# TUMFTM/CamRaDepth

Hardware: AMD Instinct MI355X
Metric: training images/sec at 256x416 bf16 (higher is better)
Workload: dtype bf16; 1 GPU; CamRaDepth base (image+radar) train step, 8x7x256x416 per GPU, bf16 MFMA / fp32 accumulate, diffGradNorm + OneCycleLR, Dropout2d/DropPath on; global_batch=8, parallelism=dp1, hip_graph=True

## Files before the change

camradepth_amd/csrc/encoder_ops.hip:

```cpp
#include <stdlib.h>
#include "common.h"

namespace {

constexpr int TPB = 256;

constexpr int DTH = 8;
constexpr int DCW = 64;

struct InNorm {
  const crd_sum_t* stats;
  const float* gamma; const float* beta; int gmul;
};
__device__ __forceinline__ void innorm_coeffs(const InNorm& n, int b, int C, long long P, int c0, bool ok, float (&a)[8], float (&s)[8]) {
#pragma unroll
  for (int j = 0; j < 8; ++j) { a[j] = 1.f; s[j] = 0.f; }
  if (n.stats == nullptr || !ok) return;
  float mean, rstd;
  const int grp = (c0 >> 4) / n.gmul;
  gn_mean_rstd(n.stats + (long long)b * (C >> 4) * 2, grp * n.gmul, n.gmul, (float)P * 16.f * n.gmul, mean, rstd);
#pragma unroll
  for (int j = 0; j < 8; ++j) {
    a[j] = n.gamma[c0 + j] * rstd;
    s[j] = n.beta[c0 + j] - mean * a[j];
// ... 97 lines not shown
  float s = 0.f, ss = 0.f;
  float rs0[8], rs1[8], rmean = 0.f, rrstd = 0.f;
#pragma unroll
  for (int j = 0; j < 8; ++j) rs0[j] = rs1[j] = 0.f;
  if (red.xr && gok) gn_mean_rstd(red.stats + (long long)b * (C >> 4) * 2, c0 >> 4, 1, (float)H * W * 16.f, rmean, rrstd);
#pragma unroll
  for (int i = 0; i < ROWS; ++i) {
#pragma unroll
    for (int kx = 0; kx < 3; ++kx) lds8(r0 + i + 2, xc + kx, win[(i + 2) % 3][kx]);
    const int oy = ty0 + r0 + i, ox = tx0 + xc;
    f32x2 acc[4];
#pragma unroll
    for (int q = 0; q < 4; ++q) acc[q] = bv[q];
#pragma unroll
    for (int ky = 0; ky < 3; ++ky)
#pragma unroll
      for (int kx = 0; kx < 3; ++kx) {
#pragma unroll
        for (int q = 0; q < 4; ++q) acc[q] = __builtin_elementwise_fma(win[(i + ky) % 3][kx][q], wv[ky * 3 + kx][q], acc[q]);
      }
    if (gok && oy < H && ox < W) {
      uint4 u;
      u.x = pack_bf2(acc[0][0], acc[0][1]); u.y = pack_bf2(acc[1][0], acc[1][1]); u.z = pack_bf2(acc[2][0], acc[2][1]); u.w = pack_bf2(acc[3][0], acc[3][1]);
      *reinterpret_cast<uint4*>(yb + ((long long)oy * W + ox) * C + c0) = u;
      if (red.xr) {
        const uint4 xv = xrv[i];
        const float gq[8] = {bf_lo(u.x), bf_hi(u.x), bf_lo(u.y), bf_hi(u.y), bf_lo(u.z), bf_hi(u.z), bf_lo(u.w), bf_hi(u.w)};
        const float xq[8] = {bf_lo(xv.x), bf_hi(xv.x), bf_lo(xv.y), bf_hi(xv.y), bf_lo(xv.z), bf_hi(xv.z), bf_lo(xv.w), bf_hi(xv.w)};
#pragma unroll
        for (int j = 0; j < 8; ++j) { rs0[j] += gq[j]; rs1[j] += gq[j] * ((xq[j] - rmean) * rrstd); }
      }
      if (STATS) {
        s += bf_lo(u.x) + bf_hi(u.x) + bf_lo(u.y) + bf_hi(u.y) + bf_lo(u.z) + bf_hi(u.z) + bf_lo(u.w) + bf_hi(u.w);
        ss += bf_lo(u.x) * bf_lo(u.x) + bf_hi(u.x) * bf_hi(u.x) + bf_lo(u.y) * bf_lo(u.y) + bf_hi(u.y) * bf_hi(u.y) +
              bf_lo(u.z) * bf_lo(u.z) + bf_hi(u.z) * bf_hi(u.z) + bf_lo(u.w) * bf_lo(u.w) + bf_hi(u.w) * bf_hi(u.w);
      }
    }
  }
  if (STATS) {
    s += __shfl_xor(s, 1); ss += __shfl_xor(ss, 1);
#pragma unroll
    for (int o = 8; o < 64; o <<= 1) { s += __shfl_xor(s, o); ss += __shfl_xor(ss, o); }
    const int wave = t >> 6, l = t & 63;
    if (l < 8 && (l & 1) == 0) { sred[wave][(l >> 1) * 2] = s; sred[wave][(l >> 1) * 2 + 1] = ss; }
    __syncthreads();
    if (t < 8) {
      const float v = sred[0][t] + sred[1][t] + sred[2][t] + sred[3][t];
      const int slab = (c_win >> 4) + (t >> 1);
      if (slab < (C >> 4)) stat_add(&stats[((long long)b * (C >> 4) + slab) * 2 + (t & 1)], v);
    }
  }
  if (red.xr) {
#pragma unroll
    for (int o = 8; o < 64; o <<= 1) {
#pragma unroll
      for (int j = 0; j < 8; ++j) { rs0[j] += __shfl_xor(rs0[j], o); rs1[j] += __shfl_xor(rs1[j], o); }
    }
    __syncthreads();
    float* fr = reinterpret_cast<float*>(sh);
    const int wave = t >> 6, l = t & 63;
    if (l < 8) {
#pragma unroll
      for (int j = 0; j < 8; ++j) { fr[wave * 128 + (l * 8 + j) * 2] = rs0[j]; fr[wave * 128 + (l * 8 + j) * 2 + 1] = rs1[j]; }
    }
    __syncthreads();
    const int nch = nG * 8;
    if (t < 2 * nch) {
      const float v = fr[t] + fr[128 + t] + fr[256 + t] + fr[384 + t];
      const int c = c_win + (t >> 1);
      grad_add(&red.r[((long long)b * C + c) * 2 + (t & 1)], v);
      fr[512 + t] = v * red.gamma[c];
    }
    __syncthreads();
    if (t < 2 * (nch >> 4)) {
      const int grp = t >> 1, which = t & 1;
      float a = 0.f;
#pragma unroll
      for (int j = 0; j < 16; ++j) a += fr[512 + (grp * 16 + j) * 2 + which];
      grad_add(&red.r[(long long)gridDim.z * C * 2 + ((long long)b * (C >> 4) + (c_win >> 4) + grp) * 2 + which], a);
    }
  }
}

#ifndef CRD_DWW_WGS
#define CRD_DWW_WGS 2
#endif
template <int TW>
__global__ __launch_bounds__(TPB, CRD_DWW_WGS) void k_dwconv_wgrad(const bf16_t* x, const bf16_t* dy, int H, int W, int C, crd_sum_t* dw10,
                                                      int replicas, int tiles_x, int tiles_y, int tiles_per_wg, InNorm inn) {
  constexpr int HWD = TW + 2;
  constexpr int HPX = (DTH + 2) * HWD;
  constexpr int RSPLIT = 32 / TW;
  constexpr int ROWS = DTH / RSPLIT;
  extern __shared__ __attribute__((aligned(16))) uint4 dsm[];
  uint4* sx = dsm;
  uint4* sdy = dsm + HPX * 8;
  const int b = blockIdx.z;
  const int c_win = blockIdx.y * DCW;
  const int txi = blockIdx.x % tiles_x, ygrp = blockIdx.x / tiles_x;
  const int tx0 = txi * TW;
  const bf16_t* xb = x + (long long)b * H * W * C;
  const bf16_t* db = dy + (long long)b * H * W * C;
  const int t = threadIdx.x;
  const int nG = (C - c_win) >= DCW ? 8 : (C - c_win) >> 3;
  const int g = t & 7, xc = (t >> 3) % TW, rg = (t >> 3) / TW;
  float acc[10][8];
#pragma unroll
  for (int tp = 0; tp < 10; ++tp)
#pragma unroll
    for (int j = 0; j < 8; ++j) acc[tp][j] = 0.f;
  float na[8], ns[8];
  for (int it = 0; it < tiles_per_wg; ++it) {
    const int tyi = ygrp * tiles_per_wg + it;
    if (tyi >= tiles_y) break;
    const int ty0 = tyi * DTH;
    {
      constexpr int NX = (HPX * 8 + TPB - 1) / TPB, ND = (DTH * TW * 8) / TPB;
      uint4 rx[NX], rd[ND];
      bool inimg[NX];
#pragma unroll
      for (int k = 0; k < NX; ++k) {
        const int i = t + k * TPB;
        const int hp = i >> 3, gg = i & 7;
        const int hy = hp / HWD, hx = hp - hy * HWD;
        const int iy = ty0 - 1 + hy, ix = tx0 - 1 + hx;
        inimg[k] = i < HPX * 8 && gg < nG && (unsigned)iy < (unsigned)H && (unsigned)ix < (unsigned)W;
        const int cy = iy < 0 ? 0 : (iy < H ? iy : H - 1), cx = ix < 0 ? 0 : (ix < W ? ix : W - 1), cgr = gg < nG ? gg : 0;
        const uint4 u = *reinterpret_cast<const uint4*>(xb + ((long long)cy * W + cx) * C + c_win + cgr * 8);
        rx[k] = inimg[k] ? u : make_uint4(0, 0, 0, 0);
      }
#pragma unroll
      for (int k = 0; k < ND; ++k) {
        const int i = t + k * TPB;
        const int pp = i >> 3, gg = i & 7;
        const int py = pp / TW, px = pp - py * TW;
        const int iy = ty0 + py, ix = tx0 + px;
        const int cy = iy < H ? iy : H - 1, cx = ix < W ? ix : W - 1, cgr = gg < nG ? gg : 0;
        const uint4 u = *reinterpret_cast<const uint4*>(db + ((long long)cy * W + cx) * C + c_win + cgr * 8);
        rd[k] = (gg < nG && iy < H && ix < W) ? u : make_uint4(0, 0, 0, 0);
      }
      if (it == 0) innorm_coeffs(inn, b, C, (long long)H * W, c_win + (t & 7) * 8, (t & 7) < nG, na, ns);
      if (it > 0) __syncthreads();
#pragma unroll
      for (int k = 0; k < NX; ++k) {
        const int i = t + k * TPB;
        if (i < HPX * 8) sx[i] = (inn.stats && inimg[k]) ? innorm_apply(rx[k], na, ns) : rx[k];
      }
#pragma unroll
      for (int k = 0; k < ND; ++k) sdy[t + k * TPB] = rd[k];
    }
    __syncthreads();
    float win[3][3][8];
    const int r0 = rg * ROWS;
#pragma unroll
    for (int ky = 0; ky < 2; ++ky)
#pragma unroll
      for (int kx = 0; kx < 3; ++kx) unpack8(sx[((r0 + ky) * HWD + xc + kx) * 8 + g], win[ky][kx]);
#pragma unroll
    for (int i = 0; i < ROWS; ++i) {
#pragma unroll
      for (int kx = 0; kx < 3; ++kx) unpack8(sx[((r0 + i + 2) * HWD + xc + kx) * 8 + g], win[(i + 2) % 3][kx]);
      float d[8];
      unpack8(sdy[((r0 + i) * TW + xc) * 8 + g], d);
#pragma unroll
      for (int j = 0; j < 8; ++j) acc[9][j] += d[j];
#pragma unroll
      for (int ky = 0; ky < 3; ++ky)
#pragma unroll
        for (int kx = 0; kx < 3; ++kx) {
#pragma unroll
          for (int j = 0; j < 8; ++j) acc[ky * 3 + kx][j] += d[j] * win[(i + ky) % 3][kx][j];
        }
    }
  }
#pragma unroll
  for (int o = 8; o < 64; o <<= 1) {
#pragma unroll
    for (int tp = 0; tp < 10; ++tp)
#pragma unroll
      for (int j = 0; j < 8; ++j) acc[tp][j] += __shfl_xor(acc[tp][j], o);
  }
  __syncthreads();
  float* sm = reinterpret_cast<float*>(dsm);
  const int wave = t >> 6, l = t & 63;
  for (int w = 0; w < 4; ++w) {
    if (wave == w && l < 8) {
#pragma unroll
      for (int tp = 0; tp < 10; ++tp)
#pragma unroll
        for (int j = 0; j < 8; ++j) {
          float* p = &sm[tp * 64 + l * 8 + j];
          *p = w == 0 ? acc[tp][j] : *p + acc[tp][j];
        }
    }
    __syncthreads();
  }
  crd_sum_t* dst = dw10 + (long long)((blockIdx.z * gridDim.x + blockIdx.x) % replicas) * 10 * C;
  const int nch = nG * 8;
  for (int i = t; i < 10 * nch; i += TPB) {
    const int tp = i / nch, cl = i - tp * nch;
    const float v = sm[tp * 64 + cl];
    if (v != 0.f) grad_add(&dst[(long long)tp * C + c_win + cl], v);
  }
}

}

static int dw_tile_width(int W) {
  static int forced = -1;
  if (forced < 0) forced = crd_dev_int("CRD_DW_TW", 0);
  if (forced == 16 || forced == 32) return forced;
  return W <= 16 ? 16 : 32;
}

extern "C" int crd_dwconv3x3(const void* x, int32_t B, int32_t H, int32_t W, int32_t C, const float* w9, const float* bias,
                             int32_t flip, void* y, crd_sum_t* stats, const crd_sum_t* in_stats, int32_t in_gmul,
                             const float* in_gamma, const float* in_beta, const void* red_x, const crd_sum_t* red_stats,
                             const float* red_gamma, crd_sum_t* red_r, crd_stream_t stream) {
  CRD_CHECK_ARG(x && w9 && y, "crd_dwconv3x3: null pointer");
  CRD_CHECK_ARG(!red_x || (red_stats && red_gamma && red_r), "crd_dwconv3x3: incomplete fused-reduce arguments");
  const RedOut red{reinterpret_cast<const bf16_t*>(red_x), red_stats, red_gamma, red_r};
  CRD_CHECK_ARG(!in_stats || (in_gamma && in_beta && in_gmul >= 1 && (C / 16) % in_gmul == 0), "crd_dwconv3x3: bad input-norm arguments");
  const InNorm inn{in_stats, in_gamma, in_beta, in_gmul};
  CRD_CHECK_ARG(C % 16 == 0, "crd_dwconv3x3: C must be a multiple of 16");
  const bf16_t* xp = reinterpret_cast<const bf16_t*>(x);
  bf16_t* yp = reinterpret_cast<bf16_t*>(y);
  hipStream_t st = as_stream(stream);
  const int tw = dw_tile_width(W);
  const int tiles_x = cdiv(W, tw), tiles_y = cdiv(H, DTH);
  dim3 grid(tiles_x * tiles_y, cdiv(C, DCW), B);
#define CRD_DW(FL, STT, TWV) hipLaunchKernelGGL((k_dwconv<FL, STT, TWV>), grid, dim3(TPB), 0, st, xp, H, W, C, w9, bias, yp, stats, tiles_x, inn, red)
  if (tw == 32) {
    if (flip) { if (stats) CRD_DW(true, true, 32); else CRD_DW(true, false, 32); }
    else { if (stats) CRD_DW(false, true, 32); else CRD_DW(false, false, 32); }
  } else {
    if (flip) { if (stats) CRD_DW(true, true, 16); else CRD_DW(true, false, 16); }
    else { if (stats) CRD_DW(false, true, 16); else CRD_DW(false, false, 16); }
  }
#undef CRD_DW
  CRD_LAUNCH_CHECK("crd_dwconv3x3");
  return CRD_OK;
}

extern "C" int crd_dwconv3x3_wgrad(const void* x, const void* dy, int32_t B, int32_t H, int32_t W, int32_t C, crd_sum_t* dw10,
                                   int32_t replicas, const crd_sum_t* in_stats, int32_t in_gmul, const float* in_gamma,
                                   const float* in_beta, crd_stream_t stream) {
  CRD_CHECK_ARG(x && dy && dw10 && replicas >= 1, "crd_dwconv3x3_wgrad: null pointer / replicas < 1");
  CRD_CHECK_ARG(!in_stats || (in_gamma && in_beta && in_gmul >= 1 && (C / 16) % in_gmul == 0), "crd_dwconv3x3_wgrad: bad input-norm arguments");
  const InNorm inn{in_stats, in_gamma, in_beta, in_gmul};
  CRD_CHECK_ARG(C % 16 == 0 && C <= 4096, "crd_dwconv3x3_wgrad: C must be a multiple of 16, <= 4096");
  const int tw = dw_tile_width(W);
  const int tiles_x = cdiv(W, tw), tiles_y = cdiv(H, DTH), wins = cdiv(C, DCW);
  int ysplit = cdiv(512, (long long)tiles_x * wins * B);
  if (ysplit > tiles_y) ysplit = tiles_y;
  if (ysplit < 1) ysplit = 1;
  const int per = cdiv(tiles_y, ysplit);
  ysplit = cdiv(tiles_y, per);
  dim3 grid(tiles_x * ysplit, wins, B);
  const bf16_t* xp = reinterpret_cast<const bf16_t*>(x);
  const bf16_t* dp = reinterpret_cast<const bf16_t*>(dy);
  hipStream_t st = as_stream(stream);
  if (tw == 32) {
    const size_t lds = (size_t)((DTH + 2) * 34 * 8 + DTH * 32 * 8) * sizeof(uint4);
    crd_reserve_lds_once<&k_dwconv_wgrad<32>>((int)lds, "k_dwconv_wgrad");
    hipLaunchKernelGGL(k_dwconv_wgrad<32>, grid, dim3(TPB), lds, st, xp, dp, H, W, C, dw10, replicas, tiles_x, tiles_y, per, inn);
  } else {
    const size_t lds = (size_t)((DTH + 2) * 18 * 8 + DTH * 16 * 8) * sizeof(uint4);
    crd_reserve_lds_once<&k_dwconv_wgrad<16>>((int)lds, "k_dwconv_wgrad");
    hipLaunchKernelGGL(k_dwconv_wgrad<16>, grid, dim3(TPB), lds, st, xp, dp, H, W, C, dw10, replicas, tiles_x, tiles_y, per, inn);
  }
  CRD_LAUNCH_CHECK("crd_dwconv3x3_wgrad");
  return CRD_OK;
}
```

camradepth_amd/lib.py:

```python
import ctypes as C
import os
import struct

import torch

_HERE = os.path.dirname(os.path.abspath(__file__))
LIB_PATH = os.environ.get("CRD_LIB") or os.path.join(_HERE, "libcamradepth_hip.so")


class CrdError(RuntimeError):
    pass


class ConvDesc(C.Structure):
    _fields_ = [
        ("x", C.c_void_p), ("x_ld", C.c_int32), ("x_coff", C.c_int32),
        ("B", C.c_int32), ("IH", C.c_int32), ("IW", C.c_int32), ("Cin", C.c_int32),
        ("w", C.c_void_p), ("Cout", C.c_int32), ("KH", C.c_int32), ("KW", C.c_int32),
        ("stride", C.c_int32), ("pad", C.c_int32), ("OH", C.c_int32), ("OW", C.c_int32),
        ("gather_mode", C.c_int32),
        ("y", C.c_void_p), ("y_ld", C.c_int32), ("y_coff", C.c_int32), ("y_f32", C.c_int32),
        ("out_mode", C.c_int32), ("patch_k", C.c_int32), ("patch_c", C.c_int32),
        ("bias", C.c_void_p), ("bias_bstride", C.c_int32), ("act", C.c_int32),
        ("res", C.c_void_p), ("res_ld", C.c_int32), ("res_scale", C.c_void_p),
# ... 26 lines not shown
        ("dw", C.c_void_p), ("dbias", C.c_void_p), ("dw_partials", C.c_void_p), ("dw_partial_capacity", C.c_int32), ("wg_budget", C.c_int32),
    ]


class WgradGroupInfo(C.Structure):
    _fields_ = [("n_problems", C.c_int32), ("n_items", C.c_int32 * 4), ("item_offset", C.c_int32 * 4), ("bytes", C.c_int64)]


class PackEntry(C.Structure):
    _fields_ = [
        ("src", C.c_void_p), ("dst_fwd", C.c_void_p), ("dst_dgrad", C.c_void_p), ("dst_scatter", C.c_void_p),
        ("cmap", C.c_void_p),
        ("Cout", C.c_int32), ("Cin_ref", C.c_int32), ("taps", C.c_int32), ("Cin_pad", C.c_int32),
        ("Cout_pad", C.c_int32), ("dst_f32", C.c_int32),
        ("dgrad_ld", C.c_int32), ("dgrad_coff", C.c_int32), ("dgrad_row0", C.c_int32), ("dgrad_rows", C.c_int32),
    ]


class MlpDesc(C.Structure):
    _fields_ = [(n, C.c_void_p) for n in ("x1", "x1_stats", "norm_gamma", "norm_beta", "w_fc1", "b_fc1", "norm1_gamma", "norm1_beta",
                                          "w9", "b_dw", "norm2_gamma", "norm2_beta", "w_fc2", "xn", "h1", "h2", "h3", "h1_stats",
                                          "h2_stats", "fc2_partials")] + \
               [(n, C.c_int32) for n in ("B", "H", "W", "C", "hidden")]


class UnpackEntry(C.Structure):
    _fields_ = [
        ("src", C.c_void_p), ("dst", C.c_void_p), ("cmap", C.c_void_p),
        ("Cout", C.c_int32), ("Cin_ref", C.c_int32), ("taps", C.c_int32), ("Cin_pad", C.c_int32),
        ("replicas", C.c_int32), ("src_sum", C.c_int32), ("replica_stride", C.c_int64),
    ]


class DgnDesc(C.Structure):
    _fields_ = [(n, C.c_void_p) for n in ("p", "g", "exp_avg", "exp_avg_sq", "prev_grad", "exp_grad_norm", "factor", "parts", "seg_off",
                                          "blk2seg", "blk2chunk", "active", "hp_dev", "gate", "clip", "ema")] + \
               [("parts_stride", C.c_int64), ("n_tensors", C.c_int32), ("n_blocks", C.c_int32)] + \
               [(n, C.c_float) for n in ("lr", "beta1", "beta2", "eps", "weight_decay")] + \
               [("step", C.c_int32), ("max_norm", C.c_float), ("ema_decay", C.c_float),
                ("ema_warmup", C.c_int32), ("ema_n", C.c_int32), ("ema_base", C.c_int32)]


_lib = None
ABI_VERSION = 13


def load():
    global _lib
    if _lib is not None:
        return _lib
    if not os.path.exists(LIB_PATH):
        raise CrdError(f"{LIB_PATH} is missing: run `python -m camradepth_amd.build` (hipcc, gfx950). "
                       "camradepth_amd has no CPU fallback.")
    lib = C.CDLL(LIB_PATH)
    lib.crd_last_error.restype = C.c_char_p
    lib.crd_arch.restype = C.c_char_p
    lib.crd_version.restype = C.c_int
    if lib.crd_version() != ABI_VERSION:
        raise CrdError(f"{LIB_PATH} was built for ABI version {lib.crd_version()}, this binding is version {ABI_VERSION}: rebuild it "
                       "(python -m camradepth_amd.build)")
    missing = [n for n in EXPORTS if not hasattr(lib, n)]
    if missing:
        raise CrdError(f"{LIB_PATH} lacks symbols {missing}: rebuild it (python -m camradepth_amd.build)")
    for name, sig in _SIGS.items():
        fn = getattr(lib, name)
        fn.restype = C.c_int
        fn.argtypes = [_CT[ch] for ch in sig]
    if os.environ.get("CRD_DEV_SWITCHES") == "1":
        if os.environ.get("CRD_TUNE_REGE") is not None:
            lib.crd_tune_igemm_reg_epilogue(int(os.environ["CRD_TUNE_REGE"]))
        if os.environ.get("CRD_TUNE_NARROW") is not None:
            lib.crd_tune_pw_narrow(int(os.environ["CRD_TUNE_NARROW"]))
    _lib = lib
    return lib


_SIGS = {
    "crd_conv_igemm": "pp", "crd_conv_igemm_route": "ppi", "crd_gn_conv": "ppp", "crd_gn_conv2": "ppppp", "crd_gn_bwd_conv": "ppp", "crd_pw_narrow_supported": "iii", "crd_tune_pw_narrow": "i", "crd_conv3x3_fp8": "ppfp", "crd_amax_bf16": "pliiipp", "crd_quant_fp8": "pliiipiifp",
    "crd_weight_quant_fp8": "piiiippp", "crd_conv3x3_fp8_dgrad": "pppp", "crd_gn_bwd_apply_fp8": "piiipiiiiiipippipppppiipiippp",
    "crd_fp8_scale_update": "ppifip", "crd_quant_fp8_dev": "pliiipiipp", "crd_tune_conv3x3_small_grid": "i", "crd_tune_igemm_reg_epilogue": "i", "crd_conv_wgrad": "pp", "crd_conv_wgrad_splits": "p", "crd_conv_wgrad_route": "ppi", "crd_wgrad_group_build": "piplp", "crd_conv_wgrad_grouped": "ppp",
    "crd_gn_stats": "piiiiiippp", "crd_gn_apply": "piiiiiipippipPiiip".replace("P", "p"),
    "crd_gn_bwd_reduce": "piiipiiiiiipippippplp", "crd_gn_bwd_apply": "piiipiiiiiipippipppppiiiipipp",
    "crd_gn_launch_shape": "iiiippp",
    "crd_dwconv3x3": "piiiippipppippppppp", "crd_dwconv3x3_wgrad": "ppiiiipipippp",
    "crd_attn_scores": "ppiiiiifppp", "crd_attn_scores_fp8": "ppiiiiffppp", "crd_attn_fwd": "ppiiiiifpppppppppp", "crd_attn_xbar": "ppppiiipp", "crd_attn_xbar_proj": "pppppiiippp", "crd_attn_vec_bwd": "ppiiifppp", "crd_attn_out_residual": "pppppiiipp", "crd_attn_out_residual_stats": "pppppiiippp",
    "crd_attn_out_bwd": "ppppiiipppp", "crd_attn_out_bwd_blocks": "iii", "crd_attn_out_bwd_gn": "ppppiiippppppppppp", "crd_attn_scores_bwd": "ppppiiiiifpppp", "crd_attn_bwd": "ppppiiiiifpppppifppp", "crd_attn_scores_bwd_partials": "iiiii", "crd_sum_partials_bf16": "pilplp", "crd_gsum_to_bf16": "pplp",
    "crd_attn_bwd_fused_supported": "iiiii", "crd_attn_bwd_fused": "ppppppp" "iiiii" "f" "ppppp" "ppppppp" "p", "crd_attn_dk_fold": "pilpl" "pp" "iii" "f" "pp" "p",
    "crd_bicubic2x": "piiiiiipiip", "crd_bicubic2x_fp8": "piiiiiipiifpiip", "crd_gn_apply_fp8": "piiiiiipippippiifpiip", "crd_bicubic2x_bwd": "piiiiiipiiip",
    "crd_input_grad": "ppppiiiiiipp",
    "crd_nchw_to_pm": "piiiipiiip", "crd_pm_to_nchw": "piiiiiiipp", "crd_seg_argmax": "piiiiipiiip", "crd_scale_f32": "pplfp",
    "crd_slice_copy": "piipiiliip", "crd_f32_to_bf16_rows": "pipiiliplpiip", "crd_dropout_masks": "ppiiLpp", "crd_sigmoid_bwd": "pplp", "crd_head_conv2_fwd": "pppiiippiip", "crd_head_conv2_bwd": "ppiippiiippip", "crd_head_conv2_bwd_data": "ppiippiiipp", "crd_head_conv2_wgrad": "ppiipiiipip",
    "crd_weight_pack": "pilp", "crd_wgrad_unpack": "pilip",
    "crd_assemble_input": "pppiiifpp", "crd_gt_pyramid": "piiifppppp",
    "crd_augment_draw": "ppiiiiifffffffiLLp", "crd_augment_lut": "piipp", "crd_augment_assemble": "pppppppiiiiifppppp",
    "crd_augment_gather": "ppppiiiiiippppp", "crd_gt_pyramid_from_full": "piiipppp",
    "crd_radar_project": "pppiipppipiiiffpppppppp", "crd_radar_rasterize": "ppppppppiipiiiiiplppp",
    "crd_lidar_project": "pppiippppippipppipiiiffLLpppppppppp", "crd_lidar_ground_truth": "pppppppppiipiiiiipppipLplpppp",
    "crd_depth_unproject": "piiiiipipiiLLLipppppp", "crd_point_cloud": "piiiiipipiiLLLipppipplpppppp",
    "crd_bev_grid": "ppppiiipiLLLiiLLiiiplppppppp",
    "crd_occupancy_update": "pppiiipipipiiiiLiLLLLiiiiiipppppplpppppp",
    "crd_distance_field": "piiiiiippplppppp", "crd_field_paths": "pppiipLpppiiiiiippppppp",
    "crd_nav_field": "piiippipLiiipppp", "crd_nav_paths": "ppiipLppiiipppppp",
    "crd_map_objects": "piiiiiiipLplpppppp",
    "crd_track_objects": "pppp" "iiiii" "LLLL" "ii" "ppppppppp" "p",
    "crd_match_scan": "ppp" "iii" "pipi" "iii" "LLLL" "i" "ppp" "ii" "p" "il" "pl" "ppppppp" "p",
    "crd_viz_range": "piiiiipplpp", "crd_viz_draw": "piiiippffipiiffipllp", "crd_seg_labels": "piiiipp",
    "crd_camera_frontend": "piiiilliiippip",
    "crd_resize_nearest_u8":"piiiipiip", "crd_resize_labels_nearest": "piiiipiip", "crd_seg_confusion": "ppiilppp",
    "crd_masked_l1_fwd": "pplpp", "crd_test_metrics": "ppilffpp", "crd_depth_eval": "ppilfffipp", "crd_masked_l1_bwd": "pplppfpp", "crd_ce_fwd": "ppiilpp",
    "crd_ce_focal_bwd": "ppiilppfpp",
    "crd_masked_dist_fwd": "pplpp", "crd_masked_dist_bwd": "pplppfipp", "crd_masked_berhu_max": "pplppp",
    "crd_masked_berhu": "pplppLppfpp", "crd_smoothness_fwd": "ppiiiipp", "crd_smoothness_bwd": "ppiiiippfpp",
    "crd_diffgradnorm_norm": "pp", "crd_diffgradnorm_commit": "pp", "crd_diffgradnorm_step": "pp",
    "crd_mlp_fused_supported": "iiii", "crd_mlp_fwd": "pp", "crd_mlp_reduce": "pipppiiipppp",
    "crd_nonfinite_status": "ip", "crd_nonfinite_capture": "pp",
    "crd_swap_f32": "pplp",
}
_CT = {"p": C.c_void_p, "i": C.c_int32, "l": C.c_int64, "L": C.c_uint64, "f": C.c_float}
EXPORTS = list(_SIGS)


STAT_FRAC_BITS, GRAD_FRAC_BITS = 20, 44
SUM_DTYPE = torch.int64
EVAL_FRAC_BITS = (0, 32, 26, 24, 24, 36, 33, 31, 40, 0, 0, 0)
EVAL_MAX_BINS = 64
AUGMENT_WORDS, AUGMENT_STREAM = 8, 0xA0761D6478BD642F
AUGMENT_GAMMA, AUGMENT_BRIGHTNESS, AUGMENT_COLOUR = 1, 2, 4


def stat_value(t):
    return t.double() * 2.0 ** -STAT_FRAC_BITS


def grad_value(t):
    return t.double() * 2.0 ** -GRAD_FRAC_BITS


def nonfinite(reset=True):
    rc = load().crd_nonfinite_status(1 if reset else 0, stream())
    if rc < 0:
        check(rc, "crd_nonfinite_status")
    return rc == 1


def nonfinite_clear():
    check(load().crd_nonfinite_status(2, stream()), "crd_nonfinite_status")


def stat_checked(acc):
    v = stat_value(acc)
    if nonfinite(reset=False):
        v = torch.full_like(v, float("nan"))
    return v


def f64_bits(x):
    return struct.unpack("<Q", struct.pack("<d", float(x)))[0]


def check(rc, what=""):
    if rc != 0:
        msg = load().crd_last_error().decode()
        raise CrdError(f"{what} failed with status {rc}: {msg}")


def conv_route(desc):
    buf = C.create_string_buffer(96)
    check(load().crd_conv_igemm_route(C.byref(desc), buf, len(buf)), "crd_conv_igemm_route")
    return buf.value.decode()


def wgrad_route(desc):
    buf = C.create_string_buffer(96)
    check(load().crd_conv_wgrad_route(C.byref(desc), buf, len(buf)), "crd_conv_wgrad_route")
    return buf.value.decode()


def gn_launch_shape(P, Cn, B, kind):
    out = (C.c_int32 * 3)()
    ptr = [C.cast(C.byref(out, 4 * i), C.c_void_p) for i in range(3)]
    check(load().crd_gn_launch_shape(P, Cn, B, kind, *ptr), "crd_gn_launch_shape")
    return out[0], out[1], out[2]


def stream():
    return C.c_void_p(torch.cuda.current_stream().cuda_stream)


def ptr(t):
    return None if t is None else C.c_void_p(t.data_ptr())
```

include/camradepth_hip.h:

```cpp
#ifndef CAMRADEPTH_HIP_H
#define CAMRADEPTH_HIP_H

#include <stdint.h>

#ifdef __cplusplus
extern "C" {
#endif

typedef void* crd_stream_t;

#define CRD_OK 0
#define CRD_E_INVALID (-1)
#define CRD_E_UNSUPPORTED (-2)
#define CRD_E_LAUNCH (-3)

typedef int64_t crd_sum_t;
#define CRD_STAT_FRAC_BITS 20
#define CRD_GRAD_FRAC_BITS 44
int crd_nonfinite_status(int32_t reset, crd_stream_t stream);
int crd_nonfinite_capture(int32_t* window_flag, crd_stream_t stream);

const char* crd_last_error(void);
#define CRD_ABI_VERSION 13
int crd_version(void);
// ... 55 lines not shown
  const crd_sum_t* r;
  void* dx; int32_t dx_ld;
  float* dgamma; float* dbeta;
} crd_gn_bwd_input;
int crd_gn_bwd_conv(const crd_conv_desc* d, const crd_gn_bwd_input* n, crd_stream_t stream);
int crd_pw_narrow_supported(int32_t Cin, int32_t Cout, int32_t pixels);
int crd_tune_pw_narrow(int32_t on);
int crd_tune_conv3x3_small_grid(int workgroups);
int crd_tune_igemm_reg_epilogue(int32_t on);

int crd_conv3x3_fp8(const crd_conv_desc* d, const float* w_scales, float x_scale, crd_stream_t stream);
int crd_amax_bf16(const void* x, int64_t rows, int32_t ld, int32_t coff, int32_t C, float* amax, crd_stream_t stream);
int crd_quant_fp8(const void* x, int64_t rows, int32_t ld, int32_t coff, int32_t C, void* y, int32_t y_ld, int32_t y_coff,
                  float scale, crd_stream_t stream);
int crd_gn_apply_fp8(const void* x, int32_t x_f32, int32_t x_ld, int32_t x_coff, int32_t B, int32_t P, int32_t C, const crd_sum_t* stats,
                     int32_t gmul, const float* gamma, const float* beta, int32_t act, const float* mask, void* y_fp8, int32_t y_ld,
                     int32_t y_coff, float y_scale, void* y_bf16, int32_t yb_ld, int32_t yb_coff, crd_stream_t stream);
int crd_bicubic2x_fp8(const void* x, int32_t x_ld, int32_t x_coff, int32_t B, int32_t H, int32_t W, int32_t C, void* y_fp8,
                      int32_t y_ld, int32_t y_coff, float y_scale, void* y_bf16, int32_t yb_ld, int32_t yb_coff, crd_stream_t stream);
int crd_weight_quant_fp8(const void* w_bf16, int32_t Cout, int32_t taps, int32_t Cin, int32_t Cin_out, void* w_fp8, float* scales,
                         crd_stream_t stream);

int crd_conv3x3_fp8_dgrad(const crd_conv_desc* d, const float* w_scales, const float* x_scale_dev, crd_stream_t stream);
#define CRD_FP8_AMAX_SLOTS 64
int crd_gn_bwd_apply_fp8(const void* x, int32_t x_f32, int32_t x_ld, int32_t x_coff, const void* dy, int32_t dy_f32,
                         int32_t dy_ld, int32_t dy_coff, int32_t B, int32_t P, int32_t C, const crd_sum_t* stats,
                         int32_t gmul, const float* gamma, const float* beta, int32_t act, const float* mask,
                         const crd_sum_t* r, float* dgamma, float* dbeta, void* dx, int32_t dx_ld, int32_t dx_coff,
                         void* dx_fp8, int32_t dx8_ld, int32_t dx8_coff, const float* scale_dev, uint32_t* amax_slots,
                         crd_stream_t stream);
int crd_fp8_scale_update(uint32_t* amax_slots, float* scales, int32_t n, float margin, int32_t keep_slots, crd_stream_t stream);
int crd_quant_fp8_dev(const void* x, int64_t rows, int32_t ld, int32_t coff, int32_t C, void* y, int32_t y_ld, int32_t y_coff,
                      const float* scale_dev, crd_stream_t stream);

typedef struct {
  const void* x; int32_t x_ld, x_coff; int32_t B, IH, IW, Cin;
  const void* dy; int32_t dy_ld, dy_coff; int32_t OH, OW, Cout;
  int32_t KH, KW, stride, pad;
  crd_sum_t* dw;
  crd_sum_t* dbias;
  float* dw_partials;
  int32_t dw_partial_capacity;
  int32_t wg_budget;
} crd_wgrad_desc;

int crd_conv_wgrad(const crd_wgrad_desc* d, crd_stream_t stream);
int crd_conv_wgrad_splits(const crd_wgrad_desc* d);
int crd_conv_wgrad_route(const crd_wgrad_desc* d, char* label, int32_t capacity);

typedef struct crd_wgrad_group_info {
  int32_t n_problems;
  int32_t n_items[4];
  int32_t item_offset[4];
  int64_t bytes;
} crd_wgrad_group_info;
int crd_wgrad_group_build(const crd_wgrad_desc* descs, int32_t n, void* host_table, int64_t capacity,
                          crd_wgrad_group_info* info);
int crd_conv_wgrad_grouped(const void* dev_table, const crd_wgrad_group_info* info, crd_stream_t stream);

int crd_gn_stats(const void* x, int32_t x_f32, int32_t x_ld, int32_t x_coff, int32_t B, int32_t P, int32_t C,
                 crd_sum_t* stats, crd_sum_t* chan_sums, crd_stream_t stream);

int crd_gn_apply(const void* x, int32_t x_f32, int32_t x_ld, int32_t x_coff, int32_t B, int32_t P, int32_t C,
                 const crd_sum_t* stats, int32_t gmul, const float* gamma, const float* beta, int32_t act,
                 const float* mask, void* y, int32_t y_f32, int32_t y_ld, int32_t y_coff, crd_stream_t stream);

int crd_gn_bwd_reduce(const void* x, int32_t x_f32, int32_t x_ld, int32_t x_coff, const void* dy, int32_t dy_f32,
                      int32_t dy_ld, int32_t dy_coff, int32_t B, int32_t P, int32_t C, const crd_sum_t* stats,
                      int32_t gmul, const float* gamma, const float* beta, int32_t act, const float* mask,
                      crd_sum_t* r, float* scratch, int64_t scratch_capacity, crd_stream_t stream);
int crd_gn_bwd_apply(const void* x, int32_t x_f32, int32_t x_ld, int32_t x_coff, const void* dy, int32_t dy_f32,
                     int32_t dy_ld, int32_t dy_coff, int32_t B, int32_t P, int32_t C, const crd_sum_t* stats,
                     int32_t gmul, const float* gamma, const float* beta, int32_t act, const float* mask,
                     const crd_sum_t* r, float* dgamma, float* dbeta, void* dx, int32_t dx_f32, int32_t dx_ld,
                     int32_t dx_coff, int32_t dx_accumulate, void* dx2, int32_t dx2_ld, const float* scale2,
                     crd_stream_t stream);
int crd_gn_launch_shape(int32_t P, int32_t C, int32_t B, int32_t kind, int32_t* nblk, int32_t* chunk, int32_t* batch_pixels);


int crd_dwconv3x3(const void* x, int32_t B, int32_t H, int32_t W, int32_t C, const float* w9, const float* bias,
                  int32_t flip, void* y, crd_sum_t* stats, const crd_sum_t* in_stats, int32_t in_gmul, const float* in_gamma,
                  const float* in_beta, const void* red_x, const crd_sum_t* red_stats, const float* red_gamma, crd_sum_t* red_r,
                  crd_stream_t stream);
int crd_dwconv3x3_wgrad(const void* x, const void* dy, int32_t B, int32_t H, int32_t W, int32_t C, crd_sum_t* dw10,
                        int32_t replicas, const crd_sum_t* in_stats, int32_t in_gmul, const float* in_gamma,
                        const float* in_beta, crd_stream_t stream);

typedef struct {
  const float* x1; const crd_sum_t* x1_stats; const float* norm_gamma; const float* norm_beta;
  const void* w_fc1; const float* b_fc1; const float* norm1_gamma; const float* norm1_beta;
  const float* w9; const float* b_dw; const float* norm2_gamma; const float* norm2_beta;
  const void* w_fc2;
  void* xn; void* h1; void* h2; void* h3;
  crd_sum_t* h1_stats; crd_sum_t* h2_stats;
  float* fc2_partials;
  int32_t B, H, W, C, hidden;
} crd_mlp_desc;
int crd_mlp_fused_supported(int32_t H, int32_t W, int32_t C, int32_t hidden);
int crd_mlp_fwd(const crd_mlp_desc* d, crd_stream_t stream);
int crd_mlp_reduce(const float* fc2_partials, int32_t slabs, const float* x1, const float* b_fc2, const float* dp, int32_t B,
                   int32_t N, int32_t C, float* x2, crd_sum_t* stats, crd_sum_t* chan_sums, crd_stream_t stream);

int crd_attn_scores(const void* q, const void* k, int32_t B, int32_t N, int32_t M, int32_t heads, int32_t d,
                    float scale, float* S, int16_t* idx, crd_stream_t stream);
int crd_attn_scores_fp8(const void* q8, const void* k8, int32_t B, int32_t N, int32_t M, int32_t heads, float qk_scale, float scale,
                        float* ssum, int16_t* idx, crd_stream_t stream);
int crd_attn_fwd(const void* q, const void* k, int32_t B, int32_t N, int32_t M, int32_t heads, int32_t d, float scale,
                 float* S, int16_t* idx, const crd_sum_t* chan_sums, const crd_sum_t* stats, const float* gamma, const float* beta,
                 const void* w_fwd, void* xbar, float* u, crd_stream_t stream);
int crd_attn_xbar(const crd_sum_t* chan_sums, const crd_sum_t* stats, const float* gamma, const float* beta, int32_t B,
                  int32_t N, int32_t C, void* xbar, crd_stream_t stream);
int crd_attn_xbar_proj(const crd_sum_t* chan_sums, const crd_sum_t* stats, const float* gamma, const float* beta, const void* w_fwd,
                       int32_t B, int32_t N, int32_t C, void* xbar, float* u, crd_stream_t stream);
int crd_attn_vec_bwd(const crd_sum_t* t, const void* w_dgrad, int32_t B, int32_t C, int32_t Cpad, float inv_n, void* tb, float* es,
                     crd_stream_t stream);
int crd_attn_out_residual(const float* x, const float* u, const float* S, const float* bp, const float* dp,
                          int32_t B, int32_t N, int32_t C, float* x1, crd_stream_t stream);
int crd_attn_out_residual_stats(const float* x, const float* u, const float* S, const float* bp, const float* dp,
                                int32_t B, int32_t N, int32_t C, float* x1, crd_sum_t* stats, crd_stream_t stream);
int crd_attn_out_bwd(const float* dx1, const float* u, const float* S, const float* dp, int32_t B, int32_t N,
                     int32_t C, crd_sum_t* t, crd_sum_t* dbp_rows, float* dS, crd_stream_t stream);
int crd_attn_out_bwd_gn(float* dx1, const float* u, const float* S, const float* dp, int32_t B, int32_t N, int32_t C,
                        crd_sum_t* t, crd_sum_t* dbp_rows, float* dS, const float* x, const void* dxn, const crd_sum_t* stats,
                        const float* gamma, const crd_sum_t* r, float* dgamma, float* dbeta, crd_stream_t stream);
int crd_attn_out_bwd_blocks(int32_t B, int32_t N, int32_t C);
int crd_attn_scores_bwd_partials(int32_t B, int32_t N, int32_t M, int32_t heads, int32_t d);
int crd_attn_scores_bwd(const void* q, const void* k, const float* dS, const int16_t* idx, int32_t B, int32_t N,
                        int32_t M, int32_t heads, int32_t d, float scale, void* dq, crd_sum_t* dk, float* dk_partials,
                        crd_stream_t stream);
int crd_attn_bwd(const void* q, const void* k, const float* dS, const int16_t* idx, int32_t B, int32_t N, int32_t M,
                 int32_t heads, int32_t d, float scale, void* dq, crd_sum_t* dk, float* dk_partials, const crd_sum_t* t,
                 const void* w_dgrad, int32_t Cpad, float inv_n, void* tb, float* es, crd_stream_t stream);
int crd_sum_partials_bf16(const float* part, int32_t replicas, int64_t replica_stride, void* dst, int64_t n,
                          crd_stream_t stream);
int crd_attn_bwd_fused_supported(int32_t B, int32_t N, int32_t M, int32_t heads, int32_t d);
int crd_attn_bwd_fused(float* dx1, const float* u, const float* S, const float* dp, const void* q, const void* k, const int16_t* idx,
                       int32_t B, int32_t N, int32_t M, int32_t heads, int32_t d, float scale, crd_sum_t* t, crd_sum_t* dbp_rows,
                       float* dS, void* dq, float* dk_partials, const float* x, const void* dxn, const crd_sum_t* stats,
                       const float* gamma, const crd_sum_t* r, float* dgamma, float* dbeta, crd_stream_t stream);
int crd_attn_dk_fold(const float* part, int32_t replicas, int64_t replica_stride, void* dst, int64_t n, const crd_sum_t* t,
                     const void* w_dgrad, int32_t B, int32_t C, int32_t Cpad, float inv_n, void* tb, float* es, crd_stream_t stream);
int crd_gsum_to_bf16(const crd_sum_t* src, void* dst, int64_t n, crd_stream_t stream);

int crd_bicubic2x(const void* x, int32_t x_ld, int32_t x_coff, int32_t B, int32_t H, int32_t W, int32_t C, void* y,
                  int32_t y_ld, int32_t y_coff, crd_stream_t stream);
int crd_bicubic2x_bwd(const void* dy, int32_t dy_ld, int32_t dy_coff, int32_t B, int32_t H, int32_t W, int32_t C,
                      void* dx, int32_t dx_ld, int32_t dx_coff, int32_t accumulate, crd_stream_t stream);

int crd_input_grad(const void* draw, const void* wpe, const void* dcb_depth, const void* dcb_seg, int32_t dcb_ld, int32_t col0,
                   int32_t B, int32_t H, int32_t W, int32_t Cin, float* dx, crd_stream_t stream);

int crd_nchw_to_pm(const float* x, int32_t B, int32_t C, int32_t H, int32_t W, void* y, int32_t y_ld, int32_t y_coff,
                   int32_t Cpad, crd_stream_t stream);
int crd_pm_to_nchw(const void* x, int32_t x_f32, int32_t x_ld, int32_t x_coff, int32_t B, int32_t C, int32_t H,
                   int32_t W, float* y, crd_stream_t stream);
int crd_seg_argmax(const void* logits, int32_t ld, int32_t B, int32_t P, int32_t C, int32_t num_classes, void* y,
                   int32_t y_f32, int32_t y_ld, int32_t y_coff, crd_stream_t stream);
int crd_scale_f32(const float* src, float* dst, int64_t n, float scale, crd_stream_t stream);
int crd_slice_copy(const void* src, int32_t s_ld, int32_t s_coff, void* dst, int32_t d_ld, int32_t d_coff,
                   int64_t rows, int32_t C, int32_t accumulate, crd_stream_t stream);
int crd_f32_to_bf16_rows(const float* src, int32_t s_ld, void* dst, int32_t d_ld, int32_t d_coff, int64_t rows,
                         int32_t C, const float* scale, int64_t rows_per_sample, const void* add, int32_t add_ld,
                         int32_t add_coff, crd_stream_t stream);
int crd_head_conv2_fwd(const void* a, const float* w, const float* bias, int32_t B, int32_t H, int32_t W, float* depth,
                       void* copy, int32_t copy_ld, int32_t copy_coff, crd_stream_t stream);
int crd_head_conv2_bwd(const float* gd, const void* add, int32_t add_ld, int32_t add_coff, const void* a, const float* w,
// ... 217 lines not shown
```

Before: 470.6 images/s.

## Add MFMA-based depthwise 3x3 conv kernel with automatic routing

Adds a depthwise 3x3 convolution kernel that maps the taps onto bf16 MFMA instructions using sparse diagonal weight fragments, with extra lo-part MFMAs to keep fp32 weight precision. Halo tiles are staged in swizzled LDS, and the fused input-norm, stats and reduce epilogues are kept. A route function enables it by default when W>16 and the grid is large enough. The aim is to move the depthwise FMA work off the VALU, at the cost of wasted MFMA lanes and possibly tripled MFMA work when weights are not bf16-exact.

```diff
diff --git a/camradepth_amd/csrc/encoder_ops.hip b/camradepth_amd/csrc/encoder_ops.hip
--- a/camradepth_amd/csrc/encoder_ops.hip
+++ b/camradepth_amd/csrc/encoder_ops.hip
@@ -203,6 +203,206 @@
   }
 }
 
+constexpr int MHW = 34;
+constexpr int MHPX = (DTH + 2) * MHW;
+
+template <bool FLIP, bool STATS, bool RED>
+__global__ __launch_bounds__(TPB, 3) void k_dwconv_mma(const bf16_t* x, int H, int W, int C, const float* w9, const float* bias,
+                                                       bf16_t* y, crd_sum_t* stats, int tiles_x, InNorm inn, RedOut red) {
+  typedef __attribute__((ext_vector_type(4))) unsigned u32x4;
+  constexpr int NT = TPB;
+  constexpr int RPW = DTH;
+  __shared__ __attribute__((aligned(16))) uint4 sh[MHPX * 8 + 1];
+  const int b = blockIdx.z;
+  const int c_win = blockIdx.y * DCW;
+  const int tyi = blockIdx.x / tiles_x, txi = blockIdx.x - tyi * tiles_x;
+  const int ty0 = tyi * DTH, tx0 = txi * 32;
+  const char* xb = reinterpret_cast<const char*>(x + (long long)b * H * W * C);
+  char* yb = reinterpret_cast<char*>(y + (long long)b * H * W * C);
+  const int t = threadIdx.x;
+  const int nG = (C - c_win) >= DCW ? 8 : (C - c_win) >> 3;
+  const int wave = t >> 6, l = t & 63;
+  const int p = l & 15, kq = l >> 4;
+  const bool wok = wave * 2 < nG;
+  const int cg = c_win + (wok ? wave * 16 : 0);
+  union Frag { bf16x8 v; unsigned u[4]; };
+  Frag wf[5];
+  float wlo[5];
+  const int wdw = (l & 7) >> 1, wsft = (l & 1) * 16;
+  bool has_lo = false;
+  f32x4 bv = {0.f, 0.f, 0.f, 0.f};
+  float na[8], ns[8];
+  innorm_coeffs(inn, b, C, (long long)H * W, c_win + (t & 7) * 8, (t & 7) < nG, na, ns);
+  float rmean = 0.f, rrstd = 0.f;
+  if (RED) gn_mean_rstd(red.stats + (long long)b * (C >> 4) * 2, cg >> 4, 1, (float)H * W * 16.f, rmean, rrstd);
+  {
+    constexpr int NP = (MHPX * 8 + NT - 1) / NT;
+    uint4 r[NP];
+    bool inimg[NP];
+#pragma unroll
+    for (int k = 0; k < NP; ++k) {
+      const int i = t + k * NT;
+      const int hp = i >> 3, g = i & 7;
+      const int hy = hp / MHW, hx = hp - hy * MHW;
+      const int iy = ty0 - 1 + hy, ix = tx0 - 1 + hx;
+      inimg[k] = i < MHPX * 8 && g < nG && (unsigned)iy < (unsigned)H && (unsigned)ix < (unsigned)W;
+      const int cy = iy < 0 ? 0 : (iy < H ? iy : H - 1), cx = ix < 0 ? 0 : (ix < W ? ix : W - 1), cgr = g < nG ? g : 0;
+      const uint4 u = *reinterpret_cast<const uint4*>(xb + (unsigned)(((cy * W + cx) * C + c_win + cgr * 8) * 2));
+      r[k] = inimg[k] ? u : make_uint4(0, 0, 0, 0);
+    }
+    if (wok) {
+      const int c = l & 15;
+#pragma unroll
+      for (int s = 0; s < 5; ++s) {
+        const int tap = 2 * s + (kq >> 1);
+        const bool nz = tap < 9 && (kq & 1) == (c >> 3);
+        const int tp = tap < 9 ? tap : 8;
+        const float w = w9[(long long)(FLIP ? 8 - tp : tp) * C + cg + c];
+        const float wv = nz ? w : 0.f;
+        const unsigned hb = pack_bf2(wv, 0.f) & 0xffffu;
+        const float lo = wv - bf_lo(hb);
+        has_lo = has_lo || lo != 0.f;
+        wlo[s] = lo;
+#pragma unroll
+        for (int d = 0; d < 4; ++d) wf[s].u[d] = d == wdw ? hb << wsft : 0u;
+      }
+      if (bias) {
+#pragma unroll
+        for (int j = 0; j < 4; ++j) bv[j] = bias[cg + 4 * kq + j];
+      }
+    }
+#pragma unroll
+    for (int k = 0; k < NP; ++k) {
+      const int i = t + k * NT;
+      const int hp = i >> 3, g = i & 7;
+      if (i < MHPX * 8) sh[hp * 8 + (g ^ (hp & 7))] = (inn.stats && inimg[k]) ? innorm_apply(r[k], na, ns) : r[k];
+    }
+    if (t == 0) sh[MHPX * 8] = make_uint4(0, 0, 0, 0);
+  }
+  has_lo = __any(has_lo);
+  const int px = tx0 + 16 * (kq & 1) + p, c8 = cg + 8 * (kq >> 1);
+  const int pxc = px < W ? px : W - 1;
+  uint4 xrv[RPW];
+  if (RED && wok) {
+    const char* xrb = reinterpret_cast<const char*>(red.xr + (long long)b * H * W * C);
+#pragma unroll
+    for (int i = 0; i < RPW; ++i) {
+      const int oy = ty0 + i;
+      const int cy = oy < H ? oy : H - 1;
+      xrv[i] = *reinterpret_cast<const uint4*>(xrb + (unsigned)(((cy * W + pxc) * C + c8) * 2));
+    }
+  }
+  __syncthreads();
+  if (!wok) return;
+  auto seg_row = [](int seg) { return (seg >> 2) + 4 * ((seg >> 1) & 1); };
+  int hpo[5];
+#pragma unroll
+  for (int s = 0; s < 5; ++s) {
+    const int tap = 2 * s + (kq >> 1);
+    const int tp = tap < 9 ? tap : 8;
+    hpo[s] = (tp / 3) * MHW + (tp % 3) + p;
+  }
+  const bool zl = kq >= 2;
+  const int gi = (wave * 2 + (kq & 1));
+  const char* shb = reinterpret_cast<const char*>(sh);
+  auto read_frags = [&](int seg, Frag (&f)[5]) {
+    const int rl = seg_row(seg), h = seg & 1;
+#pragma unroll
+    for (int s = 0; s < 5; ++s) {
+      const int sw = (hpo[s] + 2 * (rl & 3)) & 7;
+      unsigned a = (unsigned)(hpo[s] * 128 + ((gi ^ sw) << 4)) + (unsigned)((rl * MHW + 16 * h) * 128);
+      if (s == 4) a = zl ? (unsigned)(MHPX * 128) : a;
+      f[s].v = *reinterpret_cast<const bf16x8*>(shb + a);
+    }
+  };
+  const bool h1 = tx0 + 16 < W;
+  float s1 = 0.f, s2 = 0.f;
+  float rs0[8], rs1[8];
+#pragma unroll
+  for (int j = 0; j < 8; ++j) rs0[j] = rs1[j] = 0.f;
+  Frag cur[5], nxt[5];
+  f32x4 acc0;
+  read_frags(0, cur);
+#pragma unroll
+  for (int seg = 0; seg < 2 * RPW; ++seg) {
+    const bool live = (seg & 1) == 0 || h1, live_next = (seg & 1) == 1 || h1;
+    if (seg + 1 < 2 * RPW && live_next) read_frags(seg + 1, nxt);
+    f32x4 acc = bv;
+    if (live) {
+#pragma unroll
+      for (int s = 0; s < 5; ++s) acc = __builtin_amdgcn_mfma_f32_16x16x32_bf16(wf[s].v, cur[s].v, acc, 0, 0, 0);
+      if (has_lo) {
+#pragma unroll
+        for (int s = 0; s < 5; ++s) {
+          const unsigned lb = pack_bf2(wlo[s], 0.f) & 0xffffu, lb2 = pack_bf2(wlo[s] - bf_lo(lb), 0.f) & 0xffffu;
+          Frag wl, wl2;
+#pragma unroll
+          for (int d = 0; d < 4; ++d) { wl.u[d] = d == wdw ? lb << wsft : 0u; wl2.u[d] = d == wdw ? lb2 << wsft : 0u; }
+          acc = __builtin_amdgcn_mfma_f32_16x16x32_bf16(wl.v, cur[s].v, acc, 0, 0, 0);
+          acc = __builtin_amdgcn_mfma_f32_16x16x32_bf16(wl2.v, cur[s].v, acc, 0, 0, 0);
+        }
+      }
+    }
+    if ((seg & 1) == 0) acc0 = acc;
+    else {
+      const int i = seg_row(seg);
+      const auto e0 = __builtin_amdgcn_permlane16_swap(pack_bf2(acc0[0], acc0[1]), pack_bf2(acc[0], acc[1]), false, false);
+      const auto e1 = __builtin_amdgcn_permlane16_swap(pack_bf2(acc0[2], acc0[3]), pack_bf2(acc[2], acc[3]), false, false);
+      const u32x4 u = {e0[0], e1[0], e0[1], e1[1]};
+      const int oy = ty0 + i;
+      if (oy < H && px < W) {
+        *reinterpret_cast<u32x4*>(yb + (unsigned)(((oy * W + px) * C + c8) * 2)) = u;
+        if (RED) {
+          const uint4 xv = xrv[i];
+          const float gq[8] = {bf_lo(u[0]), bf_hi(u[0]), bf_lo(u[1]), bf_hi(u[1]), bf_lo(u[2]), bf_hi(u[2]), bf_lo(u[3]), bf_hi(u[3])};
+          const float xq[8] = {bf_lo(xv.x), bf_hi(xv.x), bf_lo(xv.y), bf_hi(xv.y), bf_lo(xv.z), bf_hi(xv.z), bf_lo(xv.w), bf_hi(xv.w)};
+#pragma unroll
+          for (int j = 0; j < 8; ++j) { rs0[j] += gq[j]; rs1[j] += gq[j] * ((xq[j] - rmean) * rrstd); }
+        }
+        if (STATS) {
+#pragma unroll
+          for (int d = 0; d < 4; ++d) {
+            s1 += bf_lo(u[d]) + bf_hi(u[d]);
+            s2 += bf_lo(u[d]) * bf_lo(u[d]) + bf_hi(u[d]) * bf_hi(u[d]);
+          }
+        }
+      }
+    }
+#pragma unroll
+    for (int s = 0; s < 5; ++s) cur[s] = nxt[s];
+  }
+  if (STATS) {
+    s1 = wave_sum(s1); s2 = wave_sum(s2);
+    if (l < 2) stat_add(&stats[((long long)b * (C >> 4) + (cg >> 4)) * 2 + l], l ? s2 : s1);
+  }
+  if (RED) {
+    float v[16];
+#pragma unroll
+    for (int j = 0; j < 8; ++j) { v[j] = rs0[j]; v[8 + j] = rs1[j]; }
+#pragma unroll
+    for (int o = 1, n = 8; o < 16; o <<= 1, n >>= 1) {
+      const bool up = (l & o) != 0;
+#pragma unroll
+      for (int i = 0; i < n; ++i) {
+        const float keep = up ? v[2 * i + 1] : v[2 * i], send = up ? v[2 * i] : v[2 * i + 1];
+        v[i] = keep + __shfl_xor(send, o);
+      }
+    }
+    const float tot = v[0] + __shfl_xor(v[0], 16);
+    const int c = c8 + (p & 7), m = p >> 3;
+    const bool own = (kq & 1) == 0;
+    float gs = 0.f;
+    if (own) {
+      grad_add(&red.r[((long long)b * C + c) * 2 + m], tot);
+      gs = tot * red.gamma[c];
+    }
+#pragma unroll
+    for (int o = 1; o < 8; o <<= 1) gs += __shfl_xor(gs, o);
+    gs += __shfl_xor(gs, 32);
+    if ((l & 55) == 0) grad_add(&red.r[(long long)gridDim.z * C * 2 + ((long long)b * (C >> 4) + (cg >> 4)) * 2 + m], gs);
+  }
+}
+
 #ifndef CRD_DWW_WGS
 #define CRD_DWW_WGS 2
 #endif
@@ -334,6 +534,29 @@
   return W <= 16 ? 16 : 32;
 }
 
+static int g_dw_mma = -1;
+
+extern "C" int crd_tune_dwconv_mma(int mode) {
+  const int old = g_dw_mma;
+  g_dw_mma = mode < 0 ? -1 : (mode ? 1 : 0);
+  return old;
+}
+
+static bool dw_mma_supported(int B, int H, int W, int C) {
+  return B >= 1 && H >= 1 && W >= 1 && C >= 16 && C % 16 == 0 && (long long)H * W * C * 2 < (1ll << 31);
+}
+
+static bool dw_mma_default(int B, int H, int W, int C, int flip) {
+  (void)flip;
+  return W > 16 && (long long)cdiv(W, 32) * cdiv(H, DTH) * cdiv(C, DCW) * B >= 256;
+}
+
+extern "C" int crd_dwconv3x3_route(int32_t B, int32_t H, int32_t W, int32_t C, int32_t flip) {
+  if (!dw_mma_supported(B, H, W, C) || g_dw_mma == 0) return CRD_DWCONV_ROUTE_VALU;
+  if (g_dw_mma == 1) return CRD_DWCONV_ROUTE_MMA;
+  return dw_mma_default(B, H, W, C, flip) ? CRD_DWCONV_ROUTE_MMA : CRD_DWCONV_ROUTE_VALU;
+}
+
 extern "C" int crd_dwconv3x3(const void* x, int32_t B, int32_t H, int32_t W, int32_t C, const float* w9, const float* bias,
                              int32_t flip, void* y, crd_sum_t* stats, const crd_sum_t* in_stats, int32_t in_gmul,
                              const float* in_gamma, const float* in_beta, const void* red_x, const crd_sum_t* red_stats,
@@ -347,6 +570,18 @@
   const bf16_t* xp = reinterpret_cast<const bf16_t*>(x);
   bf16_t* yp = reinterpret_cast<bf16_t*>(y);
   hipStream_t st = as_stream(stream);
+  if (crd_dwconv3x3_route(B, H, W, C, flip) == CRD_DWCONV_ROUTE_MMA) {
+    const int tiles_x = cdiv(W, 32), tiles_y = cdiv(H, DTH);
+    dim3 grid(tiles_x * tiles_y, cdiv(C, DCW), B);
+#define CRD_DWM3(FL, STT, RD) hipLaunchKernelGGL((k_dwconv_mma<FL, STT, RD>), grid, dim3(TPB), 0, st, xp, H, W, C, w9, bias, yp, stats, tiles_x, inn, red)
+#define CRD_DWM(FL, STT) do { if (red.xr) CRD_DWM3(FL, STT, true); else CRD_DWM3(FL, STT, false); } while (0)
+    if (flip) { if (stats) CRD_DWM(true, true); else CRD_DWM(true, false); }
+    else { if (stats) CRD_DWM(false, true); else CRD_DWM(false, false); }
+#undef CRD_DWM3
+#undef CRD_DWM
+    CRD_LAUNCH_CHECK("crd_dwconv3x3");
+    return CRD_OK;
+  }
   const int tw = dw_tile_width(W);
   const int tiles_x = cdiv(W, tw), tiles_y = cdiv(H, DTH);
   dim3 grid(tiles_x * tiles_y, cdiv(C, DCW), B);
diff --git a/camradepth_amd/lib.py b/camradepth_amd/lib.py
--- a/camradepth_amd/lib.py
+++ b/camradepth_amd/lib.py
@@ -132,7 +132,7 @@
     "crd_gn_stats": "piiiiiippp", "crd_gn_apply": "piiiiiipippipPiiip".replace("P", "p"),
     "crd_gn_bwd_reduce": "piiipiiiiiipippippplp", "crd_gn_bwd_apply": "piiipiiiiiipippipppppiiiipipp",
     "crd_gn_launch_shape": "iiiippp",
-    "crd_dwconv3x3": "piiiippipppippppppp", "crd_dwconv3x3_wgrad": "ppiiiipipippp",
+    "crd_dwconv3x3": "piiiippipppippppppp", "crd_dwconv3x3_wgrad": "ppiiiipipippp", "crd_dwconv3x3_route": "iiiii", "crd_tune_dwconv_mma": "i",
     "crd_attn_scores": "ppiiiiifppp", "crd_attn_scores_fp8": "ppiiiiffppp", "crd_attn_fwd": "ppiiiiifpppppppppp", "crd_attn_xbar": "ppppiiipp", "crd_attn_xbar_proj": "pppppiiippp", "crd_attn_vec_bwd": "ppiiifppp", "crd_attn_out_residual": "pppppiiipp", "crd_attn_out_residual_stats": "pppppiiippp",
     "crd_attn_out_bwd": "ppppiiipppp", "crd_attn_out_bwd_blocks": "iii", "crd_attn_out_bwd_gn": "ppppiiippppppppppp", "crd_attn_scores_bwd": "ppppiiiiifpppp", "crd_attn_bwd": "ppppiiiiifpppppifppp", "crd_attn_scores_bwd_partials": "iiiii", "crd_sum_partials_bf16": "pilplp", "crd_gsum_to_bf16": "pplp",
     "crd_attn_bwd_fused_supported": "iiiii", "crd_attn_bwd_fused": "ppppppp" "iiiii" "f" "ppppp" "ppppppp" "p", "crd_attn_dk_fold": "pilpl" "pp" "iii" "f" "pp" "p",
@@ -226,6 +226,10 @@
     return buf.value.decode()
 
 
+def dwconv_route(B, H, W, Cn, flip):
+    return ("k_dwconv", "k_dwconv_mma")[load().crd_dwconv3x3_route(B, H, W, Cn, 1 if flip else 0)]
+
+
 def gn_launch_shape(P, Cn, B, kind):
     out = (C.c_int32 * 3)()
     ptr = [C.cast(C.byref(out, 4 * i), C.c_void_p) for i in range(3)]
diff --git a/include/camradepth_hip.h b/include/camradepth_hip.h
--- a/include/camradepth_hip.h
+++ b/include/camradepth_hip.h
@@ -161,6 +161,10 @@
                   int32_t flip, void* y, crd_sum_t* stats, const crd_sum_t* in_stats, int32_t in_gmul, const float* in_gamma,
                   const float* in_beta, const void* red_x, const crd_sum_t* red_stats, const float* red_gamma, crd_sum_t* red_r,
                   crd_stream_t stream);
+#define CRD_DWCONV_ROUTE_VALU 0
+#define CRD_DWCONV_ROUTE_MMA 1
+int crd_dwconv3x3_route(int32_t B, int32_t H, int32_t W, int32_t C, int32_t flip);
+int crd_tune_dwconv_mma(int mode);
 int crd_dwconv3x3_wgrad(const void* x, const void* dy, int32_t B, int32_t H, int32_t W, int32_t C, crd_sum_t* dw10,
                         int32_t replicas, const crd_sum_t* in_stats, int32_t in_gmul, const float* in_gamma,
                         const float* in_beta, crd_stream_t stream);
```

Result: no change. 472.4 images/s (median of 5 runs) (+0.4%).
